# rimelq/VISTAF-RoboSkin-Vision-Integrated-Multimodal-Sensor

Measured on AMD Instinct MI355X. Metric: frames/sec (224x224 -> force-map) at batch 256, higher is better.
Workload: dtype f32; 1 GPU; BASELINE configs[2]: batch 256/GPU of 224x224x3 fp16 fringe frames (256 distinct frames) -> 224x224 f32 depth map + force scalars, full FTP path (inpaint, demod, unwrap, detrend, compose, force tail), constants scaled-224; inputs resident in HBM; global_batch=256, input_dtype=fp16, constants=scaled, parallelism=dp1, inflight_batches=3, frames_with_nonzero_status=0

## Files before the change

vistaf-roboskin-vision-integrated-multimodal-sensor_amd/_lib.py:

```python
from __future__ import annotations

import ctypes
import os

_HERE = os.path.dirname(os.path.abspath(__file__))
LIB_PATH = os.path.join(_HERE, "libvistaf_ftp.so")

NSCALARS = 16
NREFINFO = 8
NCONTACT = 16
MAX_CONTACTS = 64
NTRACK = 16
TRACK_NAMES = ["track_id", "age_frames", "parent_row", "events", "overlap_px", "dx", "dy", "dforce_N", "dvolume_cm3", "origin_track_id"]
TRACK_EVENTS = {"born": 1, "split": 2, "merged": 4, "gated": 8}
FATE_ENDED, FATE_NO_ROW = -1, -2 ** 31
NSHAPE = 24
SHAPE_NAMES = ["contact_pixels", "boundary_pixels", "footprint_cx", "footprint_cy", "major_axis_mm", "minor_axis_mm", "orientation_rad",
               "fit_pixels", "fit_status", "apex_x", "apex_y", "apex_depth_mm", "curvature_1_per_mm", "curvature_2_per_mm",
               "curvature_axis_rad", "radius_1_mm", "radius_2_mm", "fit_rms_mm"]
SHAPE_FIT = {"ok": 0, "none": 1, "not_a_cap": 2}
NTAXEL, NTAXELFRAME, TAXEL_NONE = 12, 8, 0xFFFF
TAXEL_NAMES = ["contact_pixels", "contact_area_mm2", "volume_cm3", "mean_depth_mm", "max_depth_mm", "argmax_index", "centroid_x", "centroid_y",
               "force_N", "pressure_kPa"]
TAXEL_FRAME_NAMES = ["active_taxels", "volume_cm3", "force_N", "cop_x", "cop_y", "moment_x_Nmm", "moment_y_Nmm", "peak_taxel"]
# ... 283 lines not shown
    "vistaf_ftp_test_centreline_tier": (ci, [ci, ci]),
}
LOBES_SIGNATURES = {
    "vistaf_lobes_workspace_bytes": (ci, [ci, ci, ci, ci, P(sz)]),
    "vistaf_lobes_measure": (ci, [vp, vp, vp, vp, vp, ci, ci, ci, ci, ci, cd, cd, cd, vp, vp, vp, vp, vp, vp, vp, vp, sz, vp]),
}
LOBES_TEST_SIGNATURES = {
    "vistaf_ftp_test_lobes_tier": (ci, [ci, ci]),
}
POST_SIGNATURES = {
    "vistaf_ftp_test_smooth_reliable": (ci, [vp, vp, vp, cd, vp, ci, ci, ci, ci, vp]),
    "vistaf_ftp_test_core_flip": (ci, [vp, vp, vp, ci, ci, vp]),
    "vistaf_ftp_test_hole_candidates": (ci, [vp, vp, vp, ci, cf, cf, vp, ci, ci, ci, vp]),
    "vistaf_ftp_test_hole_tmp": (ci, [vp, vp, vp, vp, vp, ci, ci, vp]),
    "vistaf_ftp_test_hole_zin": (ci, [vp, vp, ci, ci, vp]),
    "vistaf_ftp_test_hole_merge": (ci, [vp, vp, vp, vp, vp, ci, ci, vp]),
    "vistaf_ftp_test_height_finish": (ci, [vp, vp, vp, vp, vp, vp, cf, ci, cd, ci, cd, cd, cd, ci, vp, vp, vp, vp, ci, ci, ci, ci, vp]),
    "vistaf_ftp_test_to_mm": (ci, [vp, vp, ci, cd, cd, cd, ci, vp, vp, vp, ci, ci, vp]),
    "vistaf_ftp_test_tail": (ci, [vp, vp, vp, vp, cd, cd, cd, ci, cd, cd, cd, vp, ci, vp, ci, ci, ci, vp]),
    "vistaf_ftp_test_backend": (ci, [vp, vp, vp, vp, vp, vp, vp, cd, cd, cd, cd, cd, ci, cd, cd, cd, vp, vp, vp, vp, ci, vp, vp, ci, ci, ci, ci, vp]),
    "vistaf_ftp_test_backend_fits": (ci, [ci, ci]),
    "vistaf_ftp_test_frame_records": (ci, [vp, vp, vp, vp, vp, vp, vp, ci, vp, ci, vp]),
}
EXTENSION_SIGNATURES = [MASK_CHAIN_SIGNATURES, DFT_STAGED_SIGNATURES, GAUSS_STRIP_SIGNATURES, FIT_WINDOW_SIGNATURES, OUTLINE_SIGNATURES, TEXTURE_SIGNATURES,
                        MATCH_SIGNATURES, CENTRELINE_SIGNATURES, CENTRELINE_TEST_SIGNATURES, LOBES_SIGNATURES, LOBES_TEST_SIGNATURES, POST_SIGNATURES]
(EXPORTS, ALIGN_EXPORTS, TEST_EXPORTS, TEMP_EXPORTS, TEMPMODEL_EXPORTS, TSENSOR_EXPORTS, TRACK_EXPORTS, SHAPE_EXPORTS, TAXEL_EXPORTS, THERMAL_EXPORTS,
 TEMPORAL_EXPORTS, CLOUD_EXPORTS, MOTION_EXPORTS, PRESSURE_EXPORTS) = (list(group) for group in SIGNATURES.values())

_lib = None


def load():
    global _lib
    if _lib is not None:
        return _lib
    if not os.path.exists(LIB_PATH):
        raise RuntimeError(
            f"{LIB_PATH} is missing: build it with `python __graft_entry__.py` (hipcc --offload-arch=gfx950). "
            "This package has no CPU path."
        )
    lib = ctypes.CDLL(LIB_PATH)
    for group in list(SIGNATURES.values()) + EXTENSION_SIGNATURES:
        for name, (restype, argtypes) in group.items():
            fn = getattr(lib, name)
            fn.restype, fn.argtypes = restype, argtypes
    _lib = lib
    return lib

# ... 8 lines not shown
```

vistaf-roboskin-vision-integrated-multimodal-sensor_amd/csrc/api.hip:

```cpp
#include <hip/hip_runtime.h>
#include <algorithm>
#include <cmath>
#include <cstdlib>
#include <cstring>
#include <map>
#include <string>
#include <vector>

#include "stages.hpp"
#include "mask_bits.hpp"

using namespace vf;
#include "test_hooks.h"
#ifdef VISTAF_DEBUG
namespace vf { void telea_debug_dump(); void telea_window_debug_dump(int B); void telea_window_mw_debug_dump(int B); void fit_debug_dump(); void unwrap_big_debug_dump(); void unwrap_batch_debug_dump(); }
#endif

static thread_local std::string g_err;
static int fail(int code, const std::string &msg) { g_err = msg; return code; }
namespace vf { int set_error(int code, const std::string &msg) { return fail(code, msg); } }

namespace {

struct GKern { float *d = nullptr; int k = 0; };
// ... 434 lines not shown
static int post_demod(vistaf_ftp_handle *hd, int B, float *d_height_mm, uint8_t *d_reliable, double *d_scalars, int32_t *d_status,
                      const CarrierGeom *pair_geom, hipStream_t st, const int *bad_count = nullptr)
{
    if (!bad_count) bad_count = hd->bad_count;
    const vistaf_ftp_config &c = hd->cfg;
    int h = hd->h, w = hd->w, P = hd->P;
    bool timed = hd->timing;

    if (timed) hipEventRecord(hd->ev[ST_RELIABLE], st);
    if (hd->g_qual.k) blur(hd, hd->prod, hd->quality, hd->g_qual, B, st);
    else HIPCHK(hipMemcpyAsync(hd->quality, hd->prod, (size_t)B * P * sizeof(float), hipMemcpyDeviceToDevice, st));
    const float *qual = hd->quality;
    select(hd, qual, hd->roi, 0, nullptr, false, hd->req_amp, 1, hd->amp_thr, nullptr, B, st);
    {
        const ReliableScratch ws = {hd->rel1, hd->rel2, hd->labels, hd->area, hd->rowdist, hd->dist, hd->cc_best, hd->morph_pre};
        const int tier = reliable_mask_chain(qual, hd->roi, hd->amp_thr, hd->se_close, c.valid_close_iters, c.reliable_edge_margin_px, ws,
                                             hd->tiers.chamfer_twopass != 0, hd->rel0, hd->reliable, hd->rel_count, hd->status,
                                             (hd->tiers.fused_masks & MCH_RELIABLE) != 0, B, h, w, st);
        if (tier < 0) return tier;
    }

    if (timed) hipEventRecord(hd->ev[ST_UNWRAP_RANK], st);
    launch_unwrap(hd->wrapped, qual, hd->reliable, hd->unwrapped, hd->parent, hd->unwrap_scratch, hd->status, B, h, w, st,
                  timed ? hd->ev[ST_UNWRAP_TREE] : nullptr, timed ? hd->ev[ST_UNWRAP] : nullptr, hd->tiers.big_flood_handback != 0, hd->tiers.unwrap_fast ? hd->unwrap_need : nullptr);

    if (timed) hipEventRecord(hd->ev[ST_DETREND], st);
    const bool fit_win = hd->tiers.fit_window != 0;
    if (c.plane_order_for_removal > 0) {
        const FitSecond detrend1 = {c.poly_order, 0, hd->resid0};
        launch_robust_polyfit_window(hd->unwrapped, hd->reliable, c.plane_order_for_removal, c.irls_iters, (float)c.irls_c, 200, 500, hd->coef, hd->phase1, &detrend1,
                                     hd->fit_need, fit_win, 0, B, h, w, st, chain_scratch(hd));
    } else {
        HIPCHK(hipMemcpyAsync(hd->phase1, hd->unwrapped, (size_t)B * P * sizeof(float), hipMemcpyDeviceToDevice, st));
        launch_robust_polyfit(hd->phase1, hd->reliable, c.poly_order, c.irls_iters, (float)c.irls_c, 200, 0, hd->coef, hd->resid0, B, h, w, st, chain_scratch(hd));
    }
    select(hd, hd->resid0, hd->reliable, (size_t)P, nullptr, true, hd->req_contact, 3, hd->thr3, nullptr, B, st);
    {
        const ContactScratchPlanes ws = {hd->contact, hd->cand, hd->morph_pre};
        const int tier = contact_mask_chain(hd->resid0, hd->reliable, hd->thr3, hd->rel_count, c.min_contact_frac, c.max_contact_frac, hd->se_contact,
                                            c.dilate_iters, ws, hd->contact_count, hd->thr_used, hd->contact_d, hd->background, hd->bg_count,
                                            (hd->tiers.fused_masks & MCH_CONTACT) != 0, B, h, w, st);
        if (tier < 0) return tier;
    }
    launch_robust_polyfit(hd->phase1, hd->background, c.poly_order, c.irls_iters, (float)c.irls_c, 200, 0, hd->coef, hd->detr, B, h, w, st, chain_scratch(hd));
    select(hd, hd->detr, hd->background, (size_t)P, nullptr, false, hd->req_med, 1, hd->bg_med, nullptr, B, st);

    if (timed) hipEventRecord(hd->ev[ST_SMOOTH_FLIP], st);
// ... 160 lines not shown
    hd->timing = enable != 0;
    return 0;
}
int vistaf_ftp_get_stage_times(vistaf_ftp_handle *hd, float *ms_out, int n)
{
    if (!hd || !ms_out) return fail(VISTAF_E_INVALID, "null argument");
    for (int i = 0; i < n && i < ST_COUNT; i++) ms_out[i] = hd->stage_ms[i];
    return 0;
}

int vistaf_ftp_test_set(vistaf_ftp_handle *hd, const char *name, int value)
{
    if (!hd || !name) return fail(VISTAF_E_INVALID, "null argument");
    const std::string n(name);
    if (n == "inpaint_tier" && value >= 0 && value <= 2) hd->tiers.inpaint = value;
    else if (n == "big_flood_handback") hd->tiers.big_flood_handback = value != 0;
    else if (n == "chamfer_twopass") hd->tiers.chamfer_twopass = value != 0;
    else if (n == "telea_two_tier") hd->tiers.telea_two_tier = value != 0;
    else if (n == "telea_mw") hd->tiers.telea_mw = value != 0;
    else if (n == "big_queue_lds") hd->tiers.big_queue_lds = value != 0;
    else if (n == "big_gq_cap" && (value == 0 || (value >= 64 && (value & (value - 1)) == 0))) hd->tiers.big_gq_cap = value;
    else if (n == "big_fallback") hd->tiers.big_fallback = value != 0;
    else if (n == "unwrap_fast") hd->tiers.unwrap_fast = value != 0;
    else if (n == "big_chain") hd->tiers.big_chain = value != 0;
    else if (n == "select_resident") hd->tiers.select_resident = value != 0;
    else if (n == "dft_staged") hd->tiers.dft_staged = value != 0;
    else if (n == "fused_chains") hd->tiers.fused_chains = value != 0;
    else if (n == "gauss_strip") hd->tiers.gauss_strip = value != 0;
    else if (n == "fit_window") hd->tiers.fit_window = value != 0;
    else if (n == "fused_backend") hd->tiers.fused_backend = value != 0;
    else if (n == "fused_masks" && value >= 0 && value <= 7) hd->tiers.fused_masks = value;
    else if (n == "keep_planes") hd->keep_planes = value != 0;
    else return fail(VISTAF_E_INVALID, "unknown test hook or value: " + n);
    return 0;
}

int vistaf_depth_map_to_volume(const float *d_height, const uint8_t *d_roi, int batch, int h, int w, double mm_per_px,
                               double depth_eps_mm, double *d_out, void *stream)
{
    if (!d_height || !d_out || batch < 1 || h < 1 || w < 1) return fail(VISTAF_E_INVALID, "bad argument");
    PostParams pp;
    pp.mm_per_px = mm_per_px; pp.depth_eps_mm = depth_eps_mm; pp.period_px = 0; pp.force_curve = Curve{0, 0, 0, 0};
    launch_tail(d_height, d_roi, nullptr, nullptr, pp, nullptr, 0, d_out, batch, h * w, (hipStream_t)stream);
    return launch_ok("launch");
}

// ... 11 lines not shown
```

vistaf-roboskin-vision-integrated-multimodal-sensor_amd/csrc/api_hooks.hip:

```cpp
#include <hip/hip_runtime.h>
#include <algorithm>
#include <cstdio>
#include <cstdlib>
#include <string>
#include <vector>

#include "stages.hpp"
#include "mask_bits.hpp"

using namespace vf;
#include "test_hooks.h"
#include "test_hooks_masks.h"
#include "test_hooks_dft.h"
#include "test_hooks_gauss.h"
#include "test_hooks_fit.h"
#include "test_hooks_post.h"

namespace {

int refuse(const std::string &msg) { return set_error(VISTAF_E_INVALID, msg); }

struct HookTemps {
    explicit HookTemps(void *stream) : st((hipStream_t)stream) {}
    HookTemps(const HookTemps &) = delete;
    ~HookTemps() { if (!mem.ptrs.empty()) (void)hipStreamSynchronize(st); mem.free_all(); }
    template <typename T>
    int alloc(T **p, size_t count) { return mem.alloc(p, count); }
    template <typename T>
    int upload(T **p, const std::vector<T> &host) { return mem.upload(p, host); }
    template <class Bufs, class Layout>
    int carve(Bufs *bufs, Layout layout) { void *buf = nullptr; return ensure_carved(mem, buf, bufs, layout); }
    int finish(int tier = 0)
    {
        const hipError_t e1 = hipGetLastError(), e2 = hipStreamSynchronize(st);
        mem.free_all();
        if (e1 != hipSuccess) return set_error(VISTAF_E_HIP, std::string("launch: ") + hipGetErrorString(e1));
        if (e2 != hipSuccess) return set_error(VISTAF_E_HIP, std::string("sync: ") + hipGetErrorString(e2));
        return tier;
    }
// ... 312 lines not shown
    ContactScratchPlanes ws;
    int *contact_count = nullptr;
    TRY(tmp.carve(&ws, [&](ScratchLayout &L) { return ContactScratchPlanes{L.take<uint8_t>(n), L.take<uint8_t>(n), L.take<uint16_t>(n)}; }));
    TRY(tmp.alloc(&contact_count, (size_t)B));
    const int tier = contact_mask_chain(resid, reliable, thr3, rel_count, min_frac, max_frac, se, iters, ws, contact_count, thr_used, contact_d, background,
                                        bg_count, fused != 0, B, h, w, tmp.st);
    return tier < 0 ? tier : tmp.finish(tier);
}

int vistaf_ftp_test_unwrap(const float *wrapped, const float *quality, const uint8_t *mask, float *unwrapped, int32_t *parent, int32_t *need,
                           int32_t *status, int B, int h, int w, int variant, void *stream)
{
    if (!wrapped || !quality || !mask || !unwrapped || !parent || !status || !plane_ok(B, h, w, 8)) return refuse("bad argument");
    if (!variant_012(variant)) return refuse(kVariant012);
    if (variant == 0 && (!need || !unwrap_fast_supported(h, w)))
        return refuse("variant 0: need is null, or the consistency check does not take this shape");
    HookTemps tmp(stream);
    uint8_t *scratch = nullptr;
    TRY(tmp.alloc(&scratch, unwrap_scratch_bytes(B, h, w)));
    launch_unwrap(wrapped, quality, mask, unwrapped, parent, scratch, status, B, h, w, tmp.st, nullptr, nullptr, variant == 2, variant == 0 ? need : nullptr);
    return tmp.finish(unwrap_tier(h, w, variant == 2));
}

int vistaf_ftp_test_inpaint(float *img_inout, const uint8_t *bad, int range, int round_u8, int32_t *fb, int32_t *status, int B, int h, int w, int variant,
                            void *stream)
{
    if (!img_inout || !bad || !fb || !status || !plane_ok(B, h, w, 8) || range < 1 || range > 100) return refuse("bad argument");
    if (variant < 0 || variant > 6) return refuse("variant must be 0 .. 6");
    if (round_u8 && variant != 1) return refuse("round_u8: the whole-frame kernel (variant 1) only");
    if (variant == 2 && !inpaint_window_mw_supported(range)) return refuse("variant 2: the 16-wave window kernel does not take this range");
    if ((variant == 5 || variant == 6) && !inpaint_clusters_supported(range)) return refuse("variants 5 and 6: the cluster kernels do not take this range");
    const bool dispatch = variant == 0 || variant >= 5;
    const size_t n_tel = variant <= 1 || variant >= 5 ? inpaint_scratch_bytes(B, h, w) : 0, n_cl = dispatch ? inpaint_cl_scratch_bytes(B, h, w) : 0,
                 n_win = variant != 1 ? inpaint_win_scratch_bytes(B) : 0;
    HookTemps tmp(stream);
    InpaintBuffers buf;
    TRY(tmp.carve(&buf, [&](ScratchLayout &L) {
        return InpaintBuffers{L.take<uint8_t>(n_tel), L.take<uint8_t>(n_cl), L.take<uint8_t>(n_win), L.take<int32_t>((size_t)B)};
    }));
    const int32_t *only = nullptr;
    if (dispatch) {
        Tiers tiers;
        if (variant >= 5) tiers.inpaint = 0;
        if (variant == 6) tiers.big_queue_lds = 0;
        only = inpaint_dispatch(img_inout, bad, range, tiers, true, buf, status, B, h, w, tmp.st, nullptr);
    } else if (variant == 1) launch_inpaint_telea(img_inout, bad, range, buf.scratch, status, nullptr, B, h, w, tmp.st, round_u8 != 0);
// ... 294 lines not shown
```

vistaf-roboskin-vision-integrated-multimodal-sensor_amd/csrc/k_unwrap.hip:

```cpp
#include "unwrap.hpp"

namespace vf {

__global__ __launch_bounds__(64) void k_unwrap_flood(const float *__restrict__ quality_all, const uint8_t *__restrict__ mask_all,
                                                     int32_t *__restrict__ parent_all, uint8_t *gst, uint32_t *gfq, uint32_t *gfi,
                                                     int cap, int32_t *status, int h, int w, const int32_t *__restrict__ only, const int32_t *__restrict__ need_frame)
{
    if (need_frame && !need_frame[blockIdx.x]) return;
    const int lane = threadIdx.x;
    const size_t b = blockIdx.x;
    if (only && !only[b]) return;
    const int P = h * w;
    const float *quality = quality_all + b * (size_t)P;
    const uint8_t *mask = mask_all + b * (size_t)P;
    int32_t *parent = parent_all + b * (size_t)P;
    uint32_t *fq = gfq + b * (size_t)cap, *fi = gfi + b * (size_t)cap;
    uint8_t *st = gst + b * (size_t)P;

    unsigned long long best = 0;
    for (int p = lane; p < P; p += 64) {
        st[p] = 0;
        parent[p] = -1;
        if (mask[p]) {
            unsigned long long k = argmax_key(quality[p], (unsigned)p);
// ... 154 lines not shown
    S.ppar = L.take<int32_t>(gn, 256, "ppar");
    const size_t codes = nb * (size_t)code_stride((long)S.EN);
    if (unwrap_ranked_supported(h, w)) S.rank = L.take<uint16_t>(codes, 256, "rank");
    else S.rank = L.take<uint32_t>(codes, 256, "rank");
    S.seed = L.take<int32_t>(nb, 256, "seed");
    S.nmask = L.take<int32_t>(nb, 256, "nmask");
    S.need_generic = L.take<int32_t>(nb, 256, "need_generic");
    S.pop_log = S.sort_b;
    S.frontier_q = S.sort_a;
    S.frontier_i = S.sort_a ? S.sort_a + gn : nullptr;
    S.tree_words = (unsigned long long *)S.sort_a;
    S.check = unwrap_fast_planes(L, B, h, w);
    return S;
}
size_t unwrap_scratch_bytes(int B, int h, int w, ScratchRec *rec) { ScratchLayout L(nullptr, rec); unwrap_scratch(L, B, h, w); return L.bytes(); }

int unwrap_tier(int h, int w, bool big_handback)
{
    return unwrap_tier_of(h, w, big_handback);
}

void launch_unwrap(const float *wrapped, const float *quality, const uint8_t *mask, float *unwrapped, int32_t *parent,
                   void *scratch, int32_t *status, int B, int h, int w, hipStream_t st, hipEvent_t ev_mid, hipEvent_t ev_flood, bool big_handback,
                   int32_t *need_buf)
{
    const int tier = unwrap_tier(h, w);
    const int P = h * w;
    ScratchLayout L(scratch);
    const UnwrapScratch S = unwrap_scratch(L, B, h, w);
    const size_t EN = S.EN;
    const int32_t *need = nullptr;
    if (need_buf && unwrap_fast_supported(h, w)) {
        launch_unwrap_fast(wrapped, quality, mask, unwrapped, need_buf, S.check, B, h, w, st);
        need = need_buf;
    }
    auto flood_and_tree = [&](const int32_t *only, const int32_t *ppar) {
        hipLaunchKernelGGL(k_unwrap_flood, dim3(B), dim3(64), 0, st, quality, mask, parent, S.state, S.frontier_q, S.frontier_i, P, status, h, w, only, need);
        if (ev_mid) hipEventRecord(ev_mid, st);
        hipLaunchKernelGGL(k_unwrap_tree, dim3(B), dim3(1024), 0, st, wrapped, parent, ppar, EN, S.tree_words, unwrapped, h, w, only, need);
    };
    if (tier == UWT_RANK16) {
        launch_unwrap_ranked(quality, mask, S.sort_a, S.sort_b, S.ppar, EN, (uint16_t *)S.rank, S.seed, B, h, w, st, ev_flood, need);
        if (ev_mid) hipEventRecord(ev_mid, st);
        launch_unwrap_replay(wrapped, S.pop_log, 2 * EN, S.ppar, EN, parent, unwrapped, B, h, w, st, need);
    } else if (tier == UWT_BITMAP) {
        launch_unwrap_rank32(quality, mask, S.sort_a, S.sort_b, EN, (uint32_t *)S.rank, S.seed, S.nmask, B, h, w, st, need);
        if (ev_flood) hipEventRecord(ev_flood, st);
        launch_unwrap_flood_big((uint32_t *)S.rank, S.seed, S.nmask, S.sort_a, 2 * EN, S.ppar, EN, S.need_generic, big_handback, B, h, w, st, need);
        flood_and_tree(S.need_generic, S.ppar);
    } else {
        if (ev_flood) hipEventRecord(ev_flood, st);
        flood_and_tree(nullptr, nullptr);
    }
}

}
// ... 1 lines not shown
```

vistaf-roboskin-vision-integrated-multimodal-sensor_amd/csrc/k_unwrap_fast.hip:

```cpp
#include <algorithm>
#include <cstdio>
#include "unwrap.hpp"

namespace vf {

constexpr uint32_t UF_KNOWN = 0x80000000u;
constexpr int UF_CH = 4;
constexpr int UF_PASSES = 8;
constexpr int UF_LDS_RUNS = 6144, UF_LDS_EDGES = 12288;
enum { UFC_NEDGE = 0, UFC_FAIL = 1, UFC_R = 2, UFC_N = 4 };

__device__ inline int uf_c(float wa, float wb, bool &tie)
{
    const float d = __fsub_rn(wb, wa), ad = fabsf(d);
    const float pi_f = 3.14159274f;
    if (ad < 6.4f) {
        tie = tie || fabsf(ad - pi_f) < 1e-5f;
        return ad > pi_f ? (d > 0.f ? -1 : 1) : 0;
    }
    const double dd = (double)wb - (double)wa;
    const int k = wrap_count(dd);
    tie = tie || fabs(fabs(dd + UW_TWOPI * (double)k) - UW_PI) < 1e-5;
    return k;
}
// ... 27 lines not shown
        return left;
    }
    __device__ int operator()(int v) { return (int)(*this)((uint32_t)v); }
    __device__ float operator()(float v) { return __uint_as_float((*this)(__float_as_uint(v))); }
};
struct Run { int index; bool start, left; };
struct RunCounter {
    LeftColumn left_on;
    int seen;
    __device__ explicit RunCounter(int first_run) : seen(first_run) {}
    __device__ Run operator()(bool on)
    {
        const int lane = threadIdx.x & 63;
        const bool left = left_on(on ? 1u : 0u) != 0u;
        const unsigned long long sb = __ballot(on && !left);
        const unsigned long long le_mask = lane == 63 ? ~0ull : (2ull << lane) - 1ull;
        const Run r = {seen + (int)__popcll(sb & le_mask) - 1, on && !left, left};
        seen += (int)__popcll(sb);
        return r;
    }
};
__device__ inline void uf_fail_if(bool bad, int32_t *ctl) { if (__ballot(bad) && (threadIdx.x & 63) == 0) ctl[UFC_FAIL] = 1; }

__global__ __launch_bounds__(1024) void k_uf_count(const float *__restrict__ quality_all, const uint8_t *__restrict__ mask_all, UfPlanes U, int h, int w, int rw)
{
    __shared__ unsigned long long s_best[16];
    const int lane = threadIdx.x & 63, wave = threadIdx.x >> 6, nwv = blockDim.x >> 6;
    const size_t b = blockIdx.y;
    const size_t P = (size_t)h * w;
    unsigned long long best = 0;
    uf_wave_rows(h, rw, [&](int y) {
        const float *q = quality_all + b * P + (size_t)y * w;
        const uint8_t *m = mask_all + b * P + (size_t)y * w;
        RunCounter runs(0);
        uint8_t mm[UF_CH];
        float qq[UF_CH];
        uf_row_chunks(
            w, [&](int j, int x) { mm[j] = x < w ? m[x] : (uint8_t)0; qq[j] = x < w ? q[x] : 0.f; },
            [&](int j, int x) {
                const bool on = mm[j] != 0;
                runs(on);
                const unsigned long long key = ((unsigned long long)f2key(qq[j]) << 32) | (uint32_t)(0x7fffffff - (y * w + x));
                if (on && key > best) best = key;
            });
        if (lane == 0) U.rowbase[b * U.hp + y + 1] = runs.seen;
    });
    best = wave_max_u64(best);
    if (lane == 0) s_best[wave] = best;
    __syncthreads();
    if (threadIdx.x == 0) {
        for (int i = 1; i < nwv; i++) best = s_best[i] > best ? s_best[i] : best;
        if (best) atomicMax(&U.seedkey[b], best);
    }
}

__global__ __launch_bounds__(1024) void k_uf_scan(UfPlanes U, int h)
{
    __shared__ int s_w[16];
    __shared__ int s_carry;
    const int tid = threadIdx.x, lane = tid & 63, wave = tid >> 6;
    const size_t b = blockIdx.x;
    int32_t *rb = U.rowbase + b * U.hp;
    if (tid == 0) { s_carry = 0; rb[0] = 0; }
    __syncthreads();
    for (int y0 = 1; y0 <= h; y0 += 1024) {
        const int y = y0 + tid;
        const int v = y <= h ? rb[y] : 0;
        const int incl = (int)wave_scan_add((uint32_t)v);
        if (lane == 63) s_w[wave] = incl;
        __syncthreads();
        int base = s_carry;
        for (int i = 0; i < wave; i++) base += s_w[i];
        if (y <= h) rb[y] = base + incl;
        __syncthreads();
        if (tid == 1023) s_carry = base + incl;
        __syncthreads();
    }
    if (tid == 0) {
        const int R = s_carry;
        U.ctl[b * UFC_N + UFC_NEDGE] = 0;
        U.ctl[b * UFC_N + UFC_R] = R;
        U.ctl[b * UFC_N + UFC_FAIL] = R > U.rcap ? 1 : 0;
    }
}

__global__ __launch_bounds__(1024) void k_uf_rows(const float *__restrict__ wrapped_all, const uint8_t *__restrict__ mask_all, UfPlanes U, int h, int w, int rw)
{
    const int lane = threadIdx.x & 63;
    const size_t b = blockIdx.y;
    if (U.ctl[b * UFC_N + UFC_FAIL]) return;
    const size_t P = (size_t)h * w;
    const size_t ro = b * (size_t)U.rcap;
    bool bad = false;
    uf_wave_rows(h, rw, [&](int y) {
        const float *wr = wrapped_all + b * P + (size_t)y * w;
        const uint8_t *m = mask_all + b * P + (size_t)y * w;
        int8_t *kk = U.kk + b * U.P16 + (size_t)y * w;
        RunCounter runs(U.rowbase[b * U.hp + y]);
        LeftColumn left_w;
        int carry_v = 0;
        uint8_t mm[UF_CH];
        float ww[UF_CH];
        uf_row_chunks(
            w, [&](int j, int x) { mm[j] = x < w ? m[x] : (uint8_t)0; ww[j] = x < w ? wr[x] : 0.f; },
            [&](int j, int x) {
// ... 180 lines not shown
    });
    uf_fail_if(bad, U.ctl + b * UFC_N);
}

__global__ __launch_bounds__(256) void k_uf_plane(const float *__restrict__ wrapped_all, float *__restrict__ unwrapped_all, UfPlanes U, int32_t *__restrict__ need, int P)
{
    const size_t b = blockIdx.y;
    const int fail = U.ctl[b * UFC_N + UFC_FAIL];
    if (blockIdx.x == 0 && threadIdx.x == 0) need[b] = fail ? 1 : 0;
    if (fail) return;
    const int p = (blockIdx.x * 256 + threadIdx.x) * 4;
    if (p >= P) return;
    const float *wr = wrapped_all + b * (size_t)P;
    float *out = unwrapped_all + b * (size_t)P;
    const int8_t *kk = U.kk + b * U.P16;
#pragma unroll
    for (int u = 0; u < 4; u++) {
        if (p + u >= P) break;
        const int kp = kk[p + u];
        out[p + u] = kp > -127 ? unwrap_value(wr[p + u], kp) : nanf32();
    }
}

UfPlanes unwrap_fast_planes(ScratchLayout &L, int B, int h, int w)
{
    UfPlanes U;
    U.rcap = std::min(60000, std::max(4096, 8 * h));
    U.ecap = std::min(65000, 2 * U.rcap);
    U.P16 = ((size_t)h * w + 15) & ~(size_t)15;
    U.hp = ((size_t)h + 2 + 3) & ~(size_t)3;
    const size_t nb = (size_t)B, nr = (size_t)U.rcap * nb, ne = (size_t)U.ecap * nb;
    U.kk = L.take<int8_t>(U.P16 * nb, 256, "check.kk");
    U.rowbase = L.take<int32_t>(U.hp * nb, 256, "check.rowbase");
    U.rstate = L.take<uint32_t>(nr, 256, "check.rstate");
    U.ei = L.take<uint16_t>(ne, 256, "check.ei");
    U.ej = L.take<uint16_t>(ne, 256, "check.ej");
    U.ed = L.take<int16_t>(ne, 256, "check.ed");
    U.seedkey = L.take<unsigned long long>(nb, 256, "check.seedkey");
    U.ctl = L.take<int32_t>(nb * UFC_N, 256, "check.ctl");
    return U;
}
bool unwrap_fast_supported(int h, int w) { return h >= 2 && w >= 2 && h <= 32767 && w <= 65535 && (long long)h * w < 0x7fffffffLL; }

void launch_unwrap_fast(const float *wrapped, const float *quality, const uint8_t *mask, float *unwrapped, int32_t *need, const UfPlanes &U, int B, int h, int w,
                        hipStream_t st)
{
    (void)hipMemsetAsync(U.seedkey, 0, (size_t)8 * B, st);
    const int rw = (long long)B * h >= 65536 ? 4 : (long long)B * h >= 16384 ? 2 : 1, nwv = 4;
    const dim3 rows((h + nwv * rw - 1) / (nwv * rw), B), blk(64 * nwv);
    hipLaunchKernelGGL(k_uf_count, rows, blk, 0, st, quality, mask, U, h, w, rw);
    hipLaunchKernelGGL(k_uf_scan, dim3(B), dim3(1024), 0, st, U, h);
    hipLaunchKernelGGL(k_uf_rows, rows, blk, 0, st, wrapped, mask, U, h, w, rw);
    hipLaunchKernelGGL(k_uf_edges, rows, blk, 0, st, wrapped, U, h, w, rw);
    static DynLdsOnce lds_once;
    const size_t lds = (size_t)UF_LDS_RUNS * 4 + (size_t)UF_LDS_EDGES * 6;
    ensure_dyn_lds(lds_once, (const void *)k_uf_propagate, (int)lds);
    hipLaunchKernelGGL(k_uf_propagate, dim3(B), dim3(1024), lds, st, U);
    hipLaunchKernelGGL(k_uf_absolute, rows, blk, 0, st, U, h, w, rw);
    hipLaunchKernelGGL(k_uf_verify, rows, blk, 0, st, wrapped, U, h, w, rw);
    const int P = h * w;
    hipLaunchKernelGGL(k_uf_plane, dim3((P + 1023) / 1024, B), dim3(256), 0, st, wrapped, unwrapped, U, need, P);
}

}
```

vistaf-roboskin-vision-integrated-multimodal-sensor_amd/csrc/kernels.hpp:

```cpp
#pragma once
#include <hip/hip_runtime.h>
#include <stdint.h>
#include <vector>
#include "common.hpp"

namespace vf {

struct Tiers {
    int inpaint = 2;
    int big_flood_handback = 0;
    int chamfer_twopass = 0;
    int telea_two_tier = 1;
    int unwrap_fast = 1;
    int big_chain = 1;
    int big_queue_lds = 1;
    int big_gq_cap = 0;
    int big_fallback = 1;
    int telea_mw = 1;
    int fused_backend = 1;
    int select_resident = 1;
    int fused_masks = 7;
    int dft_staged = 1;
    int fused_chains = 1;
    int gauss_strip = 1;
    int fit_window = 1;
};

inline bool large_frame(size_t P) { return P >= 262144; }

struct ScratchLayout;
struct ScratchRegion;
using ScratchRec = std::vector<ScratchRegion>;

struct RowSpanSE {
    int k;
    int8_t lo[33];
// ... 107 lines not shown
bool inpaint_window_mw_supported(int range);
void launch_telea_window_mw(float *img, const uint8_t *bad, const int32_t *box, int32_t *fb, int range, int B, int h, int w, hipStream_t st);
enum WindowTierAlone { WNT_ALL = 0, WNT_MW = 1, WNT_FIRST = 2 };
int32_t *launch_inpaint_window(float *img, const uint8_t *bad, int range, void *scratch, int B, int h, int w, hipStream_t st,
                               hipEvent_t ev_march = nullptr, bool two_tier = true, bool mw = true, int alone = WNT_ALL);

size_t inpaint_cl_scratch_bytes(int B, int h, int w, ScratchRec *rec = nullptr);
bool inpaint_clusters_supported(int range);
struct ClusterPlanes { const int32_t *labels, *list, *count, *xmin, *ymin, *xmax, *ymax; const uint8_t *dil; };
size_t inpaint_big_scratch_bytes(int B, int h, int w, int range = 0, ScratchRec *rec = nullptr);
bool inpaint_big_supported(int range);
void launch_inpaint_big_clusters(float *img, const uint8_t *bad_big, int range, void *scratch, int32_t *status, const ClusterPlanes &left, int B, int h,
                                 int w, hipStream_t st, bool lds_queue = true, int gq_cap = 0);
void launch_inpaint_big_handback(int32_t *status, int32_t *only, int B, hipStream_t st);
void launch_inpaint_clusters(float *img, const uint8_t *bad, int range, void *scratch, uint8_t **bad_big_out, ClusterPlanes *left, int B, int h, int w,
                             hipStream_t st);

bool unwrap_fast_supported(int h, int w);
size_t unwrap_scratch_bytes(int B, int h, int w, ScratchRec *rec = nullptr);
enum UnwrapTier { UWT_RANK16 = 0, UWT_BITMAP = 1, UWT_GENERIC = 2 };
int unwrap_tier(int h, int w, bool big_handback = false);
void launch_unwrap(const float *wrapped, const float *quality, const uint8_t *mask, float *unwrapped, int32_t *parent,
                   void *scratch, int32_t *status, int B, int h, int w, hipStream_t st, hipEvent_t ev_mid,
                   hipEvent_t ev_flood = nullptr, bool big_handback = false, int32_t *need_buf = nullptr);

void launch_robust_polyfit(const float *z, const uint8_t *mask, int order, int iters, float c, int min_count, int min_mask_count, float *coef_out,
                           float *resid_out, int B, int h, int w, hipStream_t st, void *big_scratch = nullptr);
enum FitVariant { FITV_BIG = 0, FITV_GENERIC, FITV_GENERIC_DIV, FITV_COL16, FITV_COL32, FITV_COL48, FITV_COL56, FITV_COL64, FITV_COL48_G4, FITV_COL56_G4,
                  FITV_COL64_G4, FITV_WIN16, FITV_WIN32, FITV_WIN48, FITV_WIN56, FITV_WIN32_G4, FITV_WIN48_G4, FITV_WIN56_G4, FITV_COUNT };
int polyfit_variant(int B, int h, int w, bool big, int *cols_pad_out = nullptr, int *groups_out = nullptr);
int polyfit_window_variant(int B, int h, int w, bool big);
struct FitSecond { int order, min_mask_count; float *resid_out; };
enum FitForce { FIT_WINDOW_ONLY = 1, FIT_PLAIN = 2 };
int launch_robust_polyfit_window(const float *z, const uint8_t *mask, int order, int iters, float c, int min_count, int min_mask_count, float *coef_out,
                                 float *resid_out, const FitSecond *second, int *need_flag, bool window, int force, int B, int h, int w, hipStream_t st,
                                 void *big_scratch);

void launch_zeroed_keep_nan(const float *detr, const float *bg_med, const uint8_t *reliable, float *hmap, int B, int P, hipStream_t st);
void launch_hole_candidates(const float *hmap, const uint8_t *reliable, const float *dist, int ksize, float frac_thr, float min_dist, uint8_t *cand,
                            int B, int h, int w, hipStream_t st);
void launch_hole_tmp(const float *hmap, const uint8_t *reliable, const uint8_t *cand, const float *med, float *tmp, int B, int P, hipStream_t st);
void launch_hole_zin(float *tmp_zin, const float *fill, int B, int P, hipStream_t st);
void launch_hole_merge(float *hmap, const uint8_t *reliable, const uint8_t *cand, const float *zin, uint8_t *out_rel, int B, int P, hipStream_t st);

constexpr int LAB_SHIFT = 12, LAB_SHIFT2 = 15, LAB_GAMMA_SHIFT = 3, LAB_CBRT_N = 256 * 3 / 2 * (1 << LAB_GAMMA_SHIFT);
struct LabCoef { int c[9]; int lscale, lshift; };
void launch_feature_planes(const uint8_t *bgr, const uint16_t *gamma_tab, const uint16_t *cbrt_tab, const LabCoef &cf, bool blur, float *L, float *a,
// ... 101 lines not shown
```

vistaf-roboskin-vision-integrated-multimodal-sensor_amd/csrc/unwrap.hpp:

```cpp
#pragma once
#include <cstdlib>
#include "host_util.hpp"

namespace vf {

constexpr long UW_RANK16_MAX_EN = 65533;
__host__ __device__ constexpr long padded_pixels(int h, int w) { return (long)(h + 2) * (w + 2); }
inline bool unwrap_ranked_supported(int h, int w) { return padded_pixels(h, w) <= UW_RANK16_MAX_EN; }
inline bool unwrap_big_supported(int h, int w) { return !unwrap_ranked_supported(h, w) && padded_pixels(h, w) < (1L << 26); }
inline int unwrap_tier_of(int h, int w, bool big_handback)
{
    if (unwrap_ranked_supported(h, w)) return UWT_RANK16;
    return unwrap_big_supported(h, w) && !big_handback ? UWT_BITMAP : UWT_GENERIC;
}

__host__ __device__ constexpr long code_stride(long EN) { return (EN + 7) & ~7L; }
__host__ __device__ inline int pad_index(int y, int x, int W2) { return (y + 1) * W2 + x + 1; }
inline uint32_t padded_magic(int h, int w)
{
    const unsigned long long EN = (unsigned long long)padded_pixels(h, w), W2 = (unsigned long long)w + 2;
    return EN * W2 < 0x100000000ull ? (uint32_t)(0x100000000ull / W2) + 1u : 0u;
}
__host__ __device__ inline int padded_row(int idx, uint32_t magic, int W2)
{
// ... 30 lines not shown
    const double dd = d + UW_TWOPI * k;
    if (dd <= -UW_PI) k += 1.0;
    else if (dd > UW_PI) k -= 1.0;
    return (int)k;
}
__host__ __device__ inline float unwrap_value(float w, int k) { return (float)((double)w + UW_TWOPI * (double)k); }

template <int LEVELS>
__device__ inline void bitmap_push(uint32_t r, unsigned long long *L0, unsigned long long *L1, unsigned long long *L2 = nullptr)
{
    static_assert(LEVELS == 2 || LEVELS == 3, "two or three levels");
    atomicOr(&L0[r >> 6], 1ull << (r & 63u));
    atomicOr(&L1[r >> 12], 1ull << ((r >> 6) & 63u));
    if (LEVELS == 3) atomicOr(&L2[r >> 18], 1ull << ((r >> 12) & 63u));
}

struct UfPlanes {
    int8_t *kk;
    int32_t *rowbase;
    uint32_t *rstate;
    uint16_t *ei, *ej;
    int16_t *ed;
    unsigned long long *seedkey;
    int32_t *ctl;
    size_t P16, hp;
    int rcap, ecap;
};
UfPlanes unwrap_fast_planes(ScratchLayout &L, int B, int h, int w);
void launch_unwrap_fast(const float *wrapped, const float *quality, const uint8_t *mask, float *unwrapped, int32_t *need, const UfPlanes &U, int B, int h, int w,
                        hipStream_t st);

void launch_unwrap_ranked(const float *quality, const uint8_t *mask, uint32_t *g0, uint32_t *g2, int32_t *ppar, size_t gstride, uint16_t *rank16,
                          int32_t *seed, int B, int h, int w, hipStream_t st, hipEvent_t ev_flood, const int32_t *need);
void launch_unwrap_rank32(const float *quality, const uint8_t *mask, uint32_t *gA, uint32_t *gB, size_t gstride, uint32_t *rank32, int32_t *seed,
                          int32_t *n_out, int B, int h, int w, hipStream_t st, const int32_t *need);
void launch_unwrap_flood_batch(const uint16_t *rank16, const int32_t *seed, const uint32_t *inv, size_t inv_stride, int32_t *ppar, size_t gstride,
                               uint32_t *order, size_t ostride, int B, int h, int w, hipStream_t st, const int32_t *need);
void launch_unwrap_replay(const float *wrapped, const uint32_t *order, size_t ostride, const int32_t *ppar, size_t gstride, int32_t *tree,
                          float *unwrapped, int B, int h, int w, hipStream_t st, const int32_t *need);
void launch_unwrap_flood_big(uint32_t *code, const int32_t *seed, const int32_t *n, const uint32_t *inv, size_t inv_stride, int32_t *ppar,
                             size_t gstride, int32_t *need_generic, bool force_generic, int B, int h, int w, hipStream_t st, const int32_t *need);

}
```

Baseline: 79290 frames/s.

## Fuse unwrap fast-path count/rows and absolute/verify/plane kernels

New measurement: 79990 frames/s (median of 6 runs). Within noise of the previous version (+0.9%).

```diff
diff --git a/vistaf-roboskin-vision-integrated-multimodal-sensor_amd/_lib.py b/vistaf-roboskin-vision-integrated-multimodal-sensor_amd/_lib.py
--- a/vistaf-roboskin-vision-integrated-multimodal-sensor_amd/_lib.py
+++ b/vistaf-roboskin-vision-integrated-multimodal-sensor_amd/_lib.py
@@ -329,8 +329,11 @@
     "vistaf_ftp_test_backend_fits": (ci, [ci, ci]),
     "vistaf_ftp_test_frame_records": (ci, [vp, vp, vp, vp, vp, vp, vp, ci, vp, ci, vp]),
 }
+UNWRAP_CHECK_SIGNATURES = {
+    "vistaf_ftp_test_unwrap_check": (ci, [vp, vp, vp, vp, vp, ci, ci, ci, ci, vp]),
+}
 EXTENSION_SIGNATURES = [MASK_CHAIN_SIGNATURES, DFT_STAGED_SIGNATURES, GAUSS_STRIP_SIGNATURES, FIT_WINDOW_SIGNATURES, OUTLINE_SIGNATURES, TEXTURE_SIGNATURES,
-                        MATCH_SIGNATURES, CENTRELINE_SIGNATURES, CENTRELINE_TEST_SIGNATURES, LOBES_SIGNATURES, LOBES_TEST_SIGNATURES, POST_SIGNATURES]
+                        MATCH_SIGNATURES, CENTRELINE_SIGNATURES, CENTRELINE_TEST_SIGNATURES, LOBES_SIGNATURES, LOBES_TEST_SIGNATURES, POST_SIGNATURES, UNWRAP_CHECK_SIGNATURES]
 (EXPORTS, ALIGN_EXPORTS, TEST_EXPORTS, TEMP_EXPORTS, TEMPMODEL_EXPORTS, TSENSOR_EXPORTS, TRACK_EXPORTS, SHAPE_EXPORTS, TAXEL_EXPORTS, THERMAL_EXPORTS,
  TEMPORAL_EXPORTS, CLOUD_EXPORTS, MOTION_EXPORTS, PRESSURE_EXPORTS) = (list(group) for group in SIGNATURES.values())
 
diff --git a/vistaf-roboskin-vision-integrated-multimodal-sensor_amd/csrc/api.hip b/vistaf-roboskin-vision-integrated-multimodal-sensor_amd/csrc/api.hip
--- a/vistaf-roboskin-vision-integrated-multimodal-sensor_amd/csrc/api.hip
+++ b/vistaf-roboskin-vision-integrated-multimodal-sensor_amd/csrc/api.hip
@@ -480,7 +480,7 @@
 
     if (timed) hipEventRecord(hd->ev[ST_UNWRAP_RANK], st);
     launch_unwrap(hd->wrapped, qual, hd->reliable, hd->unwrapped, hd->parent, hd->unwrap_scratch, hd->status, B, h, w, st,
-                  timed ? hd->ev[ST_UNWRAP_TREE] : nullptr, timed ? hd->ev[ST_UNWRAP] : nullptr, hd->tiers.big_flood_handback != 0, hd->tiers.unwrap_fast ? hd->unwrap_need : nullptr);
+                  timed ? hd->ev[ST_UNWRAP_TREE] : nullptr, timed ? hd->ev[ST_UNWRAP] : nullptr, hd->tiers.big_flood_handback != 0, hd->tiers.unwrap_fast ? hd->unwrap_need : nullptr, hd->tiers.unwrap_fused != 0);
 
     if (timed) hipEventRecord(hd->ev[ST_DETREND], st);
     const bool fit_win = hd->tiers.fit_window != 0;
@@ -687,6 +687,7 @@
     else if (n == "big_gq_cap" && (value == 0 || (value >= 64 && (value & (value - 1)) == 0))) hd->tiers.big_gq_cap = value;
     else if (n == "big_fallback") hd->tiers.big_fallback = value != 0;
     else if (n == "unwrap_fast") hd->tiers.unwrap_fast = value != 0;
+    else if (n == "unwrap_fused") hd->tiers.unwrap_fused = value != 0;
     else if (n == "big_chain") hd->tiers.big_chain = value != 0;
     else if (n == "select_resident") hd->tiers.select_resident = value != 0;
     else if (n == "dft_staged") hd->tiers.dft_staged = value != 0;
diff --git a/vistaf-roboskin-vision-integrated-multimodal-sensor_amd/csrc/api_hooks.hip b/vistaf-roboskin-vision-integrated-multimodal-sensor_amd/csrc/api_hooks.hip
--- a/vistaf-roboskin-vision-integrated-multimodal-sensor_amd/csrc/api_hooks.hip
+++ b/vistaf-roboskin-vision-integrated-multimodal-sensor_amd/csrc/api_hooks.hip
@@ -15,6 +15,7 @@
 #include "test_hooks_gauss.h"
 #include "test_hooks_fit.h"
 #include "test_hooks_post.h"
+#include "test_hooks_unwrap.h"
 
 namespace {
 
@@ -373,6 +374,19 @@
     return tmp.finish(unwrap_tier(h, w, variant == 2));
 }
 
+int vistaf_ftp_test_unwrap_check(const float *wrapped, const float *quality, const uint8_t *mask, float *unwrapped, int32_t *need, int B, int h, int w, int fused,
+                                 void *stream)
+{
+    if (!wrapped || !quality || !mask || !unwrapped || !need || !plane_ok(B, h, w, 8)) return refuse("bad argument");
+    if (fused != 0 && fused != 1) return refuse("fused must be 0 or 1");
+    if (!unwrap_fast_supported(h, w)) return refuse("the consistency check does not take this shape");
+    HookTemps tmp(stream);
+    uint8_t *scratch = nullptr;
+    TRY(tmp.alloc(&scratch, unwrap_check_scratch_bytes(B, h, w)));
+    launch_unwrap_check(wrapped, quality, mask, unwrapped, need, scratch, B, h, w, fused != 0, tmp.st);
+    return tmp.finish(0);
+}
+
 int vistaf_ftp_test_inpaint(float *img_inout, const uint8_t *bad, int range, int round_u8, int32_t *fb, int32_t *status, int B, int h, int w, int variant,
                             void *stream)
 {
diff --git a/vistaf-roboskin-vision-integrated-multimodal-sensor_amd/csrc/k_unwrap.hip b/vistaf-roboskin-vision-integrated-multimodal-sensor_amd/csrc/k_unwrap.hip
--- a/vistaf-roboskin-vision-integrated-multimodal-sensor_amd/csrc/k_unwrap.hip
+++ b/vistaf-roboskin-vision-integrated-multimodal-sensor_amd/csrc/k_unwrap.hip
@@ -200,7 +200,7 @@
 
 void launch_unwrap(const float *wrapped, const float *quality, const uint8_t *mask, float *unwrapped, int32_t *parent,
                    void *scratch, int32_t *status, int B, int h, int w, hipStream_t st, hipEvent_t ev_mid, hipEvent_t ev_flood, bool big_handback,
-                   int32_t *need_buf)
+                   int32_t *need_buf, bool check_fused)
 {
     const int tier = unwrap_tier(h, w);
     const int P = h * w;
@@ -209,7 +209,7 @@
     const size_t EN = S.EN;
     const int32_t *need = nullptr;
     if (need_buf && unwrap_fast_supported(h, w)) {
-        launch_unwrap_fast(wrapped, quality, mask, unwrapped, need_buf, S.check, B, h, w, st);
+        launch_unwrap_fast(wrapped, quality, mask, unwrapped, need_buf, S.check, B, h, w, check_fused, st);
         need = need_buf;
     }
     auto flood_and_tree = [&](const int32_t *only, const int32_t *ppar) {
diff --git a/vistaf-roboskin-vision-integrated-multimodal-sensor_amd/csrc/k_unwrap_fast.hip b/vistaf-roboskin-vision-integrated-multimodal-sensor_amd/csrc/k_unwrap_fast.hip
--- a/vistaf-roboskin-vision-integrated-multimodal-sensor_amd/csrc/k_unwrap_fast.hip
+++ b/vistaf-roboskin-vision-integrated-multimodal-sensor_amd/csrc/k_unwrap_fast.hip
@@ -73,6 +73,26 @@
 };
 __device__ inline void uf_fail_if(bool bad, int32_t *ctl) { if (__ballot(bad) && (threadIdx.x & 63) == 0) ctl[UFC_FAIL] = 1; }
 
+template <typename L, typename M, typename S>
+__device__ __attribute__((always_inline)) inline void uf_row_chunks(int w, L load, M mid, S step)
+{
+    const int lane = threadIdx.x & 63;
+    for (int c0 = 0; c0 < w; c0 += 64 * UF_CH) {
+#pragma unroll
+        for (int j = 0; j < UF_CH; j++) load(j, c0 + 64 * j + lane);
+#pragma unroll
+        for (int j = 0; j < UF_CH; j++) {
+            if (c0 + 64 * j >= w) break;
+            mid(j, c0 + 64 * j + lane);
+        }
+#pragma unroll
+        for (int j = 0; j < UF_CH; j++) {
+            if (c0 + 64 * j >= w) break;
+            step(j, c0 + 64 * j + lane);
+        }
+    }
+}
+
 __global__ __launch_bounds__(1024) void k_uf_count(const float *__restrict__ quality_all, const uint8_t *__restrict__ mask_all, UfPlanes U, int h, int w, int rw)
 {
     __shared__ unsigned long long s_best[16];
@@ -105,7 +125,7 @@
     }
 }
 
-__global__ __launch_bounds__(1024) void k_uf_scan(UfPlanes U, int h)
+__global__ __launch_bounds__(1024) void k_uf_scan(UfPlanes U, int h, int fused)
 {
     __shared__ int s_w[16];
     __shared__ int s_carry;
@@ -127,11 +147,65 @@
         if (tid == 1023) s_carry = base + incl;
         __syncthreads();
     }
+    const int R = s_carry;
     if (tid == 0) {
-        const int R = s_carry;
         U.ctl[b * UFC_N + UFC_NEDGE] = 0;
         U.ctl[b * UFC_N + UFC_R] = R;
-        U.ctl[b * UFC_N + UFC_FAIL] = R > U.rcap ? 1 : 0;
+        U.ctl[b * UFC_N + UFC_FAIL] = R > U.rcap || (fused && U.rowfail[b]) ? 1 : 0;
+    }
+    if (fused) {
+        uint32_t *rstate = U.rstate + b * (size_t)U.rcap;
+        for (int r = tid; r < R && r < U.rcap; r += 1024) rstate[r] = 0;
+    }
+}
+
+__global__ __launch_bounds__(1024) void k_uf_count_rows(const float *__restrict__ wrapped_all, const float *__restrict__ quality_all, const uint8_t *__restrict__ mask_all,
+                                                        UfPlanes U, int h, int w, int rw)
+{
+    __shared__ unsigned long long s_best[16];
+    const int lane = threadIdx.x & 63, wave = threadIdx.x >> 6, nwv = blockDim.x >> 6;
+    const size_t b = blockIdx.y;
+    const size_t P = (size_t)h * w;
+    unsigned long long best = 0;
+    bool bad = false;
+    uf_wave_rows(h, rw, [&](int y) {
+        const float *q = quality_all + b * P + (size_t)y * w, *wr = wrapped_all + b * P + (size_t)y * w;
+        const uint8_t *m = mask_all + b * P + (size_t)y * w;
+        int8_t *kk = U.kk + b * U.P16 + (size_t)y * w;
+        RunCounter runs(0);
+        LeftColumn left_w;
+        int carry_v = 0;
+        uint8_t mm[UF_CH];
+        float qq[UF_CH], ww[UF_CH];
+        uf_row_chunks(
+            w, [&](int j, int x) { mm[j] = x < w ? m[x] : (uint8_t)0; qq[j] = x < w ? q[x] : 0.f; ww[j] = x < w ? wr[x] : 0.f; },
+            [&](int j, int x) {
+                const bool on = mm[j] != 0;
+                const Run run = runs(on);
+                const unsigned long long key = ((unsigned long long)f2key(qq[j]) << 32) | (uint32_t)(0x7fffffff - (y * w + x));
+                if (on && key > best) best = key;
+                const float wl = left_w(ww[j]);
+                int v = 0;
+                if (on && run.left) v = uf_c(wl, ww[j], bad);
+                const uint32_t ps = wave_scan_add((uint32_t)v);
+                const uint32_t sl = wave_scan_max(run.start ? (uint32_t)lane + 1u : 0u);
+                const uint32_t pstart = (uint32_t)__builtin_amdgcn_ds_bpermute((int)((sl ? sl - 1u : 0u) << 2), (int)ps);
+                v = sl ? (int)(ps - pstart) : (int)ps + carry_v;
+                if (x < w) {
+                    if (on) bad = bad || v < -126 || v > 126;
+                    kk[x] = on ? (int8_t)v : (int8_t)-128;
+                }
+                carry_v = __builtin_amdgcn_readlane(v, 63);
+            });
+        if (lane == 0) U.rowbase[b * U.hp + y + 1] = runs.seen;
+    });
+    if (__ballot(bad) && lane == 0) U.rowfail[b] = 1;
+    best = wave_max_u64(best);
+    if (lane == 0) s_best[wave] = best;
+    __syncthreads();
+    if (threadIdx.x == 0) {
+        for (int i = 1; i < nwv; i++) best = s_best[i] > best ? s_best[i] : best;
+        if (best) atomicMax(&U.seedkey[b], best);
     }
 }
 
@@ -358,6 +432,68 @@
     }
 }
 
+__global__ __launch_bounds__(1024) void k_uf_finish(const float *__restrict__ wrapped_all, float *__restrict__ unwrapped_all, UfPlanes U, int h, int w, int rw)
+{
+    const size_t b = blockIdx.y;
+    if (U.ctl[b * UFC_N + UFC_FAIL]) return;
+    const size_t P = (size_t)h * w;
+    const uint32_t *rstate = U.rstate + b * (size_t)U.rcap;
+    bool bad = false;
+    auto absolute = [&](int8_t rel, uint32_t st) {
+        if (rel == -128) return 0u;
+        if (!(st & UF_KNOWN)) return 1u;
+        const int v = (int)rel + (int)(int16_t)(uint16_t)st;
+        if (v < -126 || v > 126) { bad = true; return 1u; }
+        return (uint32_t)(v + 128);
+    };
+    uf_wave_rows(h, rw, [&](int y) {
+        const bool dn = y + 1 < h;
+        const float *w0 = wrapped_all + b * P + (size_t)y * w, *w1 = w0 + w;
+        const int8_t *k0 = U.kk + b * U.P16 + (size_t)y * w, *k1 = k0 + w;
+        float *out = unwrapped_all + b * P + (size_t)y * w;
+        RunCounter runs0(U.rowbase[b * U.hp + y]), runs1(dn ? U.rowbase[b * U.hp + y + 1] : 0);
+        LeftColumn left_k0, left_k1, left_w0, left_w1;
+        int8_t r0[UF_CH], r1[UF_CH];
+        float ww0[UF_CH], ww1[UF_CH];
+        uint32_t st0[UF_CH], st1[UF_CH];
+        uf_row_chunks(
+            w,
+            [&](int j, int x) {
+                r0[j] = x < w ? k0[x] : (int8_t)-128;
+                ww0[j] = x < w ? w0[x] : 0.f;
+                r1[j] = dn && x < w ? k1[x] : (int8_t)-128;
+                ww1[j] = dn && x < w ? w1[x] : 0.f;
+            },
+            [&](int j, int) {
+                const bool on0 = r0[j] != -128, on1 = r1[j] != -128;
+                const Run a0 = runs0(on0), a1 = runs1(on1);
+                st0[j] = on0 ? rstate[a0.index] : 0u;
+                st1[j] = on1 ? rstate[a1.index] : 0u;
+            },
+            [&](int j, int x) {
+                const uint32_t ka = absolute(r0[j], st0[j]), kb = absolute(r1[j], st1[j]);
+                const uint32_t pka = left_k0(ka), pkb = left_k1(kb);
+                const float pw0 = left_w0(ww0[j]), pw1 = left_w1(ww1[j]);
+                auto pair = [&](uint32_t kp, uint32_t kn, float wp, float wn) {
+                    if (kp == 0 || kn == 0) return;
+                    if (kp == 1 && kn == 1) return;
+                    const int c = uf_c(wp, wn, bad);
+                    bad = bad || kp == 1 || kn == 1 || (int)kn - (int)kp != c;
+                };
+                pair(ka, kb, ww0[j], ww1[j]);
+                pair(pka, kb, pw0, ww1[j]);
+                pair(ka, pkb, ww0[j], pw1);
+                if (x < w) out[x] = ka > 1 ? unwrap_value(ww0[j], (int)ka - 128) : nanf32();
+            });
+    });
+    uf_fail_if(bad, U.ctl + b * UFC_N);
+}
+__global__ void k_uf_need(const UfPlanes U, int32_t *__restrict__ need, int B)
+{
+    const int b = blockIdx.x * blockDim.x + threadIdx.x;
+    if (b < B) need[b] = U.ctl[(size_t)b * UFC_N + UFC_FAIL] != 0 ? 1 : 0;
+}
+
 UfPlanes unwrap_fast_planes(ScratchLayout &L, int B, int h, int w)
 {
     UfPlanes U;
@@ -372,30 +508,54 @@
     U.ei = L.take<uint16_t>(ne, 256, "check.ei");
     U.ej = L.take<uint16_t>(ne, 256, "check.ej");
     U.ed = L.take<int16_t>(ne, 256, "check.ed");
-    U.seedkey = L.take<unsigned long long>(nb, 256, "check.seedkey");
+    U.seedkey = L.take<unsigned long long>(nb + (nb + 1) / 2, 256, "check.seedkey");
+    U.rowfail = U.seedkey ? (int32_t *)(U.seedkey + nb) : nullptr;
     U.ctl = L.take<int32_t>(nb * UFC_N, 256, "check.ctl");
     return U;
 }
+size_t unwrap_check_scratch_bytes(int B, int h, int w) { ScratchLayout L(nullptr); unwrap_fast_planes(L, B, h, w); return L.bytes(); }
 bool unwrap_fast_supported(int h, int w) { return h >= 2 && w >= 2 && h <= 32767 && w <= 65535 && (long long)h * w < 0x7fffffffLL; }
 
-void launch_unwrap_fast(const float *wrapped, const float *quality, const uint8_t *mask, float *unwrapped, int32_t *need, const UfPlanes &U, int B, int h, int w,
-                        hipStream_t st)
-{
-    (void)hipMemsetAsync(U.seedkey, 0, (size_t)8 * B, st);
-    const int rw = (long long)B * h >= 65536 ? 4 : (long long)B * h >= 16384 ? 2 : 1, nwv = 4;
-    const dim3 rows((h + nwv * rw - 1) / (nwv * rw), B), blk(64 * nwv);
-    hipLaunchKernelGGL(k_uf_count, rows, blk, 0, st, quality, mask, U, h, w, rw);
-    hipLaunchKernelGGL(k_uf_scan, dim3(B), dim3(1024), 0, st, U, h);
-    hipLaunchKernelGGL(k_uf_rows, rows, blk, 0, st, wrapped, mask, U, h, w, rw);
-    hipLaunchKernelGGL(k_uf_edges, rows, blk, 0, st, wrapped, U, h, w, rw);
+static void uf_launch_propagate(const UfPlanes &U, int B, hipStream_t st)
+{
     static DynLdsOnce lds_once;
     const size_t lds = (size_t)UF_LDS_RUNS * 4 + (size_t)UF_LDS_EDGES * 6;
     ensure_dyn_lds(lds_once, (const void *)k_uf_propagate, (int)lds);
     hipLaunchKernelGGL(k_uf_propagate, dim3(B), dim3(1024), lds, st, U);
+}
+void launch_unwrap_fast(const float *wrapped, const float *quality, const uint8_t *mask, float *unwrapped, int32_t *need, const UfPlanes &U, int B, int h, int w,
+                        bool fused, hipStream_t st)
+{
+    const int rw = (long long)B * h >= 65536 ? 4 : (long long)B * h >= 16384 ? 2 : 1, nwv = 4;
+    const dim3 rows((h + nwv * rw - 1) / (nwv * rw), B), blk(64 * nwv);
+    if (fused) {
+        (void)hipMemsetAsync(U.seedkey, 0, (size_t)8 * B + (size_t)4 * B, st);
+        hipLaunchKernelGGL(k_uf_count_rows, rows, blk, 0, st, wrapped, quality, mask, U, h, w, rw);
+        hipLaunchKernelGGL(k_uf_scan, dim3(B), dim3(1024), 0, st, U, h, 1);
+        hipLaunchKernelGGL(k_uf_edges, rows, blk, 0, st, wrapped, U, h, w, rw);
+        uf_launch_propagate(U, B, st);
+        hipLaunchKernelGGL(k_uf_finish, rows, blk, 0, st, wrapped, unwrapped, U, h, w, rw);
+        hipLaunchKernelGGL(k_uf_need, dim3((B + 255) / 256), dim3(256), 0, st, U, need, B);
+        return;
+    }
+    (void)hipMemsetAsync(U.seedkey, 0, (size_t)8 * B, st);
+    hipLaunchKernelGGL(k_uf_count, rows, blk, 0, st, quality, mask, U, h, w, rw);
+    hipLaunchKernelGGL(k_uf_scan, dim3(B), dim3(1024), 0, st, U, h, 0);
+    hipLaunchKernelGGL(k_uf_rows, rows, blk, 0, st, wrapped, mask, U, h, w, rw);
+    hipLaunchKernelGGL(k_uf_edges, rows, blk, 0, st, wrapped, U, h, w, rw);
+    uf_launch_propagate(U, B, st);
     hipLaunchKernelGGL(k_uf_absolute, rows, blk, 0, st, U, h, w, rw);
     hipLaunchKernelGGL(k_uf_verify, rows, blk, 0, st, wrapped, U, h, w, rw);
     const int P = h * w;
     hipLaunchKernelGGL(k_uf_plane, dim3((P + 1023) / 1024, B), dim3(256), 0, st, wrapped, unwrapped, U, need, P);
 }
 
-}
+void launch_unwrap_check(const float *wrapped, const float *quality, const uint8_t *mask, float *unwrapped, int32_t *need, void *scratch, int B, int h, int w,
+                         bool fused, hipStream_t st)
+{
+    ScratchLayout L(scratch);
+    const UfPlanes U = unwrap_fast_planes(L, B, h, w);
+    launch_unwrap_fast(wrapped, quality, mask, unwrapped, need, U, B, h, w, fused, st);
+}
+
+}
diff --git a/vistaf-roboskin-vision-integrated-multimodal-sensor_amd/csrc/kernels.hpp b/vistaf-roboskin-vision-integrated-multimodal-sensor_amd/csrc/kernels.hpp
--- a/vistaf-roboskin-vision-integrated-multimodal-sensor_amd/csrc/kernels.hpp
+++ b/vistaf-roboskin-vision-integrated-multimodal-sensor_amd/csrc/kernels.hpp
@@ -12,6 +12,7 @@
     int chamfer_twopass = 0;
     int telea_two_tier = 1;
     int unwrap_fast = 1;
+    int unwrap_fused = 1;
     int big_chain = 1;
     int big_queue_lds = 1;
     int big_gq_cap = 0;
@@ -165,7 +166,11 @@
 int unwrap_tier(int h, int w, bool big_handback = false);
 void launch_unwrap(const float *wrapped, const float *quality, const uint8_t *mask, float *unwrapped, int32_t *parent,
                    void *scratch, int32_t *status, int B, int h, int w, hipStream_t st, hipEvent_t ev_mid,
-                   hipEvent_t ev_flood = nullptr, bool big_handback = false, int32_t *need_buf = nullptr);
+                   hipEvent_t ev_flood = nullptr, bool big_handback = false, int32_t *need_buf = nullptr,
+                   bool check_fused = true);
+size_t unwrap_check_scratch_bytes(int B, int h, int w);
+void launch_unwrap_check(const float *wrapped, const float *quality, const uint8_t *mask, float *unwrapped, int32_t *need, void *scratch, int B, int h, int w,
+                         bool fused, hipStream_t st);
 
 void launch_robust_polyfit(const float *z, const uint8_t *mask, int order, int iters, float c, int min_count, int min_mask_count, float *coef_out,
                            float *resid_out, int B, int h, int w, hipStream_t st, void *big_scratch = nullptr);
diff --git a/vistaf-roboskin-vision-integrated-multimodal-sensor_amd/csrc/unwrap.hpp b/vistaf-roboskin-vision-integrated-multimodal-sensor_amd/csrc/unwrap.hpp
--- a/vistaf-roboskin-vision-integrated-multimodal-sensor_amd/csrc/unwrap.hpp
+++ b/vistaf-roboskin-vision-integrated-multimodal-sensor_amd/csrc/unwrap.hpp
@@ -76,13 +76,14 @@
     uint16_t *ei, *ej;
     int16_t *ed;
     unsigned long long *seedkey;
+    int32_t *rowfail;
     int32_t *ctl;
     size_t P16, hp;
     int rcap, ecap;
 };
 UfPlanes unwrap_fast_planes(ScratchLayout &L, int B, int h, int w);
 void launch_unwrap_fast(const float *wrapped, const float *quality, const uint8_t *mask, float *unwrapped, int32_t *need, const UfPlanes &U, int B, int h, int w,
-                        hipStream_t st);
+                        bool fused, hipStream_t st);
 
 void launch_unwrap_ranked(const float *quality, const uint8_t *mask, uint32_t *g0, uint32_t *g2, int32_t *ppar, size_t gstride, uint16_t *rank16,
                           int32_t *seed, int B, int h, int w, hipStream_t st, hipEvent_t ev_flood, const int32_t *need);
```
